# modular-ngp/phys-autodiff

Measured on NVIDIA B200. Metric: grid points/sec, fused MLP + finite-difference physics loss, higher is better.
Workload: dtype f32

## Files before the change

phys_autodiff_b200/csrc/capi.cu:

```cuda
#include "../../include/physad_b200.h"
#include "deep_grad_kernels.cuh"
#include "deep_kernels.cuh"
#include "deep_tangent_kernels.cuh"
#include "deep_tc_kernels.cuh"
#include "dense_kernels.cuh"
#include "grad_kernels.cuh"
#include "stage_kernels.cuh"
#include "tangent_grad_kernels.cuh"
#include "tangent_kernels.cuh"

#include <algorithm>
#include <cstdio>
#include <cstdlib>
#include <cstring>
#include <string>
#include <unordered_map>
#include <vector>

using namespace physad;

namespace {

thread_local std::string g_err;

int fail(int code, const std::string& msg) {
    g_err = msg;
    return code;
}

#define CU(expr)                                                                                   \
    do {                                                                                           \
        cudaError_t e_ = (expr);                                                                   \
        if (e_ != cudaSuccess)                                                                     \
            return fail(int(e_), std::string(#expr) + ": " + cudaGetErrorString(e_));              \
    } while (0)

}

struct physad_ctx {
    int device = 0;
    int sm_count = 0;
    cudaStream_t stream = nullptr;
    physad_mlp_config cfg{4, 0, 4, 1};
    bool has_weights = false;
// ... 93 lines not shown
    physad_slab r{0, g->nz};
    if (s) r = *s;
    if (r.z_begin < 0 || r.z_end > g->nz || r.z_begin > r.z_end) return fail(PHYSAD_E_INVALID, "slab outside the grid");
    *out = r;
    return 0;
}

float inv2(float h) { return float(1.0 / (2.0 * double(h))); }
double inv2d(float h) { return 1.0 / (2.0 * double(h)); }

int template_h(int H) { return H <= 32 ? 32 : (H <= 64 ? 64 : (H <= 128 ? 128 : 0)); }

template <int H>
void fill_const(const physad_ctx* c, const float tcoord[3], MlpConst<H>& k) {
    const int h_rt = c->cfg.H;
    auto W1 = [&](int h, int col) { return h < h_rt ? c->W1[size_t(h) * 4 + col] : 0.f; };
    auto B1 = [&](int h) { return h < h_rt ? c->b1[h] : 0.f; };
    auto W2 = [&](int o, int h) { return h < h_rt ? c->W2[size_t(o) * h_rt + h] : 0.f; };
    auto PT = [&](int h, int s) { volatile float p = W1(h, 3) * tcoord[s]; return float(p); };
    for (int q = 0; q < H / 2; ++q) {
        const int h0 = 2 * q, h1 = 2 * q + 1;
        k.b1p[q] = make_float2(B1(h0), B1(h1));
        k.w0s[q] = make_float2(W1(h1, 0), W1(h0, 0));
        k.w1s[q] = make_float2(W1(h1, 1), W1(h0, 1));
        k.w2s[q] = make_float2(W1(h1, 2), W1(h0, 2));
        k.ptm[q] = make_float2(PT(h0, 0), PT(h1, 0));
        k.pt0[q] = make_float2(PT(h0, 1), PT(h1, 1));
        k.ptp[q] = make_float2(PT(h0, 2), PT(h1, 2));
    }
    for (int h = 0; h < H; ++h) k.w2[h] = make_float4(W2(1, h), W2(0, h), W2(3, h), W2(2, h));
    k.b2 = make_float4(c->b2[0], c->b2[1], c->b2[2], c->b2[3]);
}

float time_coord(float t, int norm) { return norm == 1 ? t : (t + 0.5f); }

int need_4x4(const physad_ctx* c, const char* what) {
    if (!c->has_weights) return fail(PHYSAD_E_NOWEIGHTS, std::string(what) + ": no weights set");
    if (c->cfg.In != 4 || c->cfg.Out != 4)
        return fail(PHYSAD_E_UNSUPPORTED, std::string(what) + ": grid paths need In = Out = 4 (src/mlp_grid.cpp:69-80)");
    if (template_h(c->cfg.H) == 0) return fail(PHYSAD_E_UNSUPPORTED, std::string(what) + ": H > 128 not built");
    return 0;
}

float host_axis_coord(int i, int n, bool m1p1) {
    if (n <= 1) return 0.0f;
    volatile float u = float(i) / float(n - 1);
    volatile float two_u = 2.f * u;
    return m1p1 ? two_u - 1.f : float(u);
}

int ensure_coord_tables(physad_ctx* c, const physad_grid* g, cudaStream_t st) {
    const int key[5] = {g->nx, g->ny, g->nz, c->cfg.norm, 1};
    auto& t = c->tab;
    if (std::memcmp(key, t.key, sizeof(key)) == 0) return 0;
    const bool m1p1 = c->cfg.norm == 1;
    const size_t nf = size_t(g->nx) + g->ny + g->nz;
    std::vector<float> host(nf);
    for (int i = 0; i < g->nx; ++i) host[i] = host_axis_coord(i, g->nx, m1p1);
    for (int i = 0; i < g->ny; ++i) host[g->nx + i] = host_axis_coord(i, g->ny, m1p1);
    for (int i = 0; i < g->nz; ++i) host[g->nx + g->ny + i] = host_axis_coord(i, g->nz, m1p1);
    if (nf > t.cap) {
        if (t.dev) CU(cudaFree(t.dev));
        t.dev = nullptr; t.cap = 0;
        CU(cudaMalloc(&t.dev, nf * sizeof(float)));
        t.cap = nf;
    }
// ... 43 lines not shown

int build_fused_plan(physad_ctx* c, const physad_grid* g, const physad_slab& s, int TX, int TY, long long slots,
                     cudaStream_t st) {
    if (int rc = ensure_coord_tables(c, g, st)) return rc;
    auto& p = c->plan;
    p.cxs = c->tab.dev;
    p.cys = p.cxs + g->nx;
    p.czs = p.cys + g->ny;
    const int key[10] = {g->nx, g->ny, g->nz, s.z_begin, s.z_end, c->cfg.norm, TX, TY, int(slots), 1};
    if (std::memcmp(key, p.key, sizeof(key)) == 0) return 0;
    const int tiles = ((g->nx + TX - 1) / TX) * ((g->ny + TY - 1) / TY), nzl = s.z_end - s.z_begin;
    const long long want = std::min<long long>(slots, (long long)tiles * nzl);
    const std::vector<int> ranges = balanced_ranges(tiles, nzl, want, 0.9);
    const size_t bytes = ranges.size() * sizeof(int);
    if (bytes > p.cap) {
        if (p.dev) CU(cudaFree(p.dev));
        p.dev = nullptr; p.cap = 0;
        CU(cudaMalloc(&p.dev, bytes));
        p.cap = bytes;
    }
    CU(cudaMemcpyAsync(p.dev, ranges.data(), bytes, cudaMemcpyHostToDevice, st));
    CU(cudaStreamSynchronize(st));
    p.ranges = reinterpret_cast<const int*>(p.dev);
    p.blocks = int(ranges.size()) - 1;
    std::memcpy(p.key, key, sizeof(key));
    return 0;
}

template <int H, int P, int TYB, int UNROLL, int MINB, bool PACKED, bool SPLITBAR, bool DPRES>
int launch_fused_d(physad_ctx* c, const physad_grid* g, const physad_slab& s, const float tc[3], bool xchg, double* acc,
                   float* const R[4], cudaStream_t st, int blocks_per_sm_cap = 0) {
    constexpr int TX = 32, TY = TYB * P;
    auto kern = k_fused_mlp_phys_loss<H, P, TYB, UNROLL, MINB, PACKED, SPLITBAR, DPRES>;
    const size_t smem = size_t(4) * 4 * (TX + 2) * (TY + 2) * sizeof(float);
    static const long long env_blocks = getenv("PHYSAD_FUSED_BLOCKS") ? atoll(getenv("PHYSAD_FUSED_BLOCKS")) : 0;
    int& per_sm = c->blocks_per_sm[reinterpret_cast<const void*>(kern)];
    if (per_sm == 0) {
        CU(cudaFuncSetAttribute(kern, cudaFuncAttributeMaxDynamicSharedMemorySize, int(smem)));
        int q = 0;
        CU(cudaOccupancyMaxActiveBlocksPerMultiprocessor(&q, kern, 32 * TYB, smem));
        if (q < 1) return fail(PHYSAD_E_UNSUPPORTED, "fused kernel does not fit on an SM");
        per_sm = q;
    }
    const int tiles_x = (g->nx + TX - 1) / TX, tiles_y = (g->ny + TY - 1) / TY;
    const int bps = blocks_per_sm_cap > 0 ? std::min(per_sm, blocks_per_sm_cap) : per_sm;
    const long long slots = env_blocks > 0 ? env_blocks : (long long)bps * c->sm_count;
    if (int rc = build_fused_plan(c, g, s, TX, TY, slots, st)) return rc;
    const long long blocks = c->plan.blocks;
    FusedArgs a{};
    a.nx = g->nx; a.ny = g->ny; a.nz = g->nz;
    a.z_begin = s.z_begin; a.z_end = s.z_end;
    a.tiles_x = tiles_x; a.tiles_y = tiles_y;
    a.cxs = c->plan.cxs; a.cys = c->plan.cys; a.czs = c->plan.czs; a.ranges = c->plan.ranges;
    a.m1p1 = c->cfg.norm == 1; a.periodic = g->periodic != 0;
    a.inv2dt = inv2(g->dt); a.inv2hx = inv2(g->hx); a.inv2hy = inv2(g->hy); a.inv2hz = inv2(g->hz);
    a.inv2dt_d = inv2d(g->dt); a.inv2hx_d = inv2d(g->hx); a.inv2hy_d = inv2d(g->hy); a.inv2hz_d = inv2d(g->hz);
    if (int rc = ensure_partials(c, size_t(blocks))) return rc;
    a.partials = c->partials; a.ticket = c->ticket; a.acc_out = acc;
    for (int k = 0; k < 4; ++k) a.R[k] = R[k];
    if (xchg) {
        a.x.rank = c->xrank; a.x.world = c->xworld; a.x.epoch = c->xepoch + 1;
        for (int p = 0; p < XCHG_MAX_RANKS; ++p) a.x.peer[p] = c->xpeer[p];
    }
    a.status = c->d_status;
    if (c->want_host_seq) { a.host_res = c->d_res; a.host_seq = c->want_host_seq; }
    if (c->trace && blocks <= c->trace_blocks) a.trace = c->trace;
    MlpConst<H> k;
    fill_const<H>(c, tc, k);
    kern<<<unsigned(blocks), 32 * TYB, smem, st>>>(k, a);
    CU(cudaGetLastError());
    c->launches++;
    if (xchg) c->xepoch++;
    return 0;
}

template <int H, int P, int TYB, int UNROLL, int MINB, bool PACKED, bool SPLITBAR = false>
int launch_fused_t(physad_ctx* c, const physad_grid* g, const physad_slab& s, const float tc[3], bool xchg, double* acc,
                   float* const R[4], cudaStream_t st, int blocks_per_sm_cap = 0) {
    return launch_fused_d<H, P, TYB, UNROLL, MINB, PACKED, SPLITBAR, false>(c, g, s, tc, xchg, acc, R, st, blocks_per_sm_cap);
}

template <int H, bool DPRES>
int launch_fused_default(physad_ctx* c, const physad_grid* g, const physad_slab& s, const float tc[3], bool xchg,
                         double* acc, float* const R[4], cudaStream_t st) {
    const long long tile_planes = (long long)((g->nx + 31) / 32) * ((g->ny + 63) / 64) * (s.z_end - s.z_begin);
    if (tile_planes < 12LL * c->sm_count)
        return launch_fused_d<H, 4, 8, 2, 2, true, true, DPRES>(c, g, s, tc, xchg, acc, R, st, 1);
// ... 41 lines not shown
    switch (template_h(c->cfg.H)) {
        case 32: return launch_fused_h<32>(c, g, s, tc, xchg, acc, R, st);
        case 64: return launch_fused_h<64>(c, g, s, tc, xchg, acc, R, st);
        case 128: return launch_fused_h<128>(c, g, s, tc, xchg, acc, R, st);
    }
    return fail(PHYSAD_E_UNSUPPORTED, "H > 128 not built");
}

template <int H, bool FIELDS>
int launch_grid_t(physad_ctx* c, const physad_grid* g, const physad_slab& s, const float tc[3], GridInferArgs a,
                  cudaStream_t st, int dtype = PHYSAD_F32) {
    const int nzl = s.z_end - s.z_begin;
    if (nzl == 0) return 0;
    if (nzl > 65535) return fail(PHYSAD_E_UNSUPPORTED, "grid MLP kernels: more than 65535 planes per call");
    if (int rc = ensure_coord_tables(c, g, st)) return rc;
    a.cxs = c->tab.dev; a.cys = a.cxs + g->nx; a.czs = a.cys + g->ny;
    MlpConst<H> k;
    fill_const<H>(c, tc, k);
    const dim3 grid(unsigned((g->nx + 31) / 32), unsigned((g->ny + 31) / 32), unsigned(nzl));
    if (FIELDS && dtype == PHYSAD_F16) k_mlp_grid<H, FIELDS, 2, __half><<<grid, 256, 0, st>>>(k, a);
    else if (FIELDS && dtype == PHYSAD_BF16) k_mlp_grid<H, FIELDS, 2, __nv_bfloat16><<<grid, 256, 0, st>>>(k, a);
    else k_mlp_grid<H, FIELDS, 2><<<grid, 256, 0, st>>>(k, a);
    c->launches++;
    CU(cudaGetLastError());
    return 0;
}

template <bool FIELDS>
int launch_grid(physad_ctx* c, const physad_grid* g, const physad_slab& s, const float tc[3], GridInferArgs a,
                cudaStream_t st, int dtype = PHYSAD_F32) {
    a.nx = g->nx; a.ny = g->ny; a.nz = g->nz;
    a.z_begin = s.z_begin; a.z_end = s.z_end;
    a.m1p1 = c->cfg.norm == 1;
    switch (template_h(c->cfg.H)) {
        case 32: return launch_grid_t<32, FIELDS>(c, g, s, tc, a, st, dtype);
        case 64: return launch_grid_t<64, FIELDS>(c, g, s, tc, a, st, dtype);
        case 128: return launch_grid_t<128, FIELDS>(c, g, s, tc, a, st, dtype);
    }
    return fail(PHYSAD_E_UNSUPPORTED, "H > 128 not built");
}

template <bool WRITE_R, bool REDUCE, bool SCALE>
int launch_phys(physad_ctx* c, const physad_grid* g_in, PhysArgs a, cudaStream_t st, int slab_planes = -1, int dtype = PHYSAD_F32) {
    physad_grid gl = *g_in;
    if (slab_planes >= 0) gl.nz = slab_planes;
    const physad_grid* g = &gl;
    if (g->nz == 0) {
        if (REDUCE) CU(cudaMemsetAsync(a.acc_out, 0, 2 * sizeof(double), st));
        return 0;
    }
    a.nx = g->nx; a.ny = g->ny; a.nz = g->nz; a.periodic = g->periodic != 0;
    a.inv2dt = inv2(g->dt); a.inv2hx = inv2(g->hx); a.inv2hy = inv2(g->hy); a.inv2hz = inv2(g->hz);
    a.inv2dt_d = inv2d(g->dt); a.inv2hx_d = inv2d(g->hx); a.inv2hy_d = inv2d(g->hy); a.inv2hz_d = inv2d(g->hz);
    a.inv1hx_d = 1.0 / double(g->hx); a.inv1hy_d = 1.0 / double(g->hy); a.inv1hz_d = 1.0 / double(g->hz);
    a.inv1hx = float(a.inv1hx_d); a.inv1hy = float(a.inv1hy_d); a.inv1hz = float(a.inv1hz_d);
    const bool upwind = c->advection == 1;
    static const bool no_v4 = getenv("PHYSAD_NO_V4") != nullptr;
    bool v4 = !upwind && !no_v4 && g->nx % 4 == 0 && (g->nx >= 128 || dtype != PHYSAD_F32);
    const void* ptrs[12] = {a.s_m, a.s_0, a.s_p, a.u_m, a.u_0, a.u_p, a.R[0], a.R[1], a.R[2], a.R[3], a.halo_lo, a.halo_hi};
    for (int k = 0; k < 12; ++k) v4 = v4 && (uintptr_t(ptrs[k]) % ((dtype != PHYSAD_F32 && (k < 6 || k >= 10)) ? 8 : 16) == 0);
    v4 = v4 && (size_t(g->nx) * g->ny * g->nz) % 4 == 0;
    if (dtype != PHYSAD_F32 && (!v4 || SCALE || c->exact_residuals))
        return fail(PHYSAD_E_UNSUPPORTED, "16-bit fields: need nx % 4 == 0, 8-byte aligned arrays, the central scheme and fp32 residual arithmetic");
    if (v4) {
        const unsigned tx = unsigned((g->nx + 255) / 256), ty = unsigned((g->ny + V4_THREADS / 64 - 1) / (V4_THREADS / 64));
        if (ty > 65535u) return fail(PHYSAD_E_UNSUPPORTED, "phys kernels: ny > 131070");
// ... 1584 lines not shown
```

phys_autodiff_b200/csrc/fused_loss.cuh:

```cuda
#pragma once
#include <type_traits>

#include "mlp_eval.cuh"

namespace physad {

constexpr int XCHG_MAX_RANKS = 8;

struct XSlot {
    double a, b;
    unsigned long long flag;
    unsigned long long pad;
};

struct XchgArgs {
    int rank, world;
    unsigned long long epoch;
    XSlot* peer[XCHG_MAX_RANKS];
};

__device__ __forceinline__ void st_release_sys(unsigned long long* p, unsigned long long v) {
    asm volatile("st.release.sys.global.u64 [%0], %1;" ::"l"(p), "l"(v) : "memory");
}
__device__ __forceinline__ unsigned long long ld_acquire_sys(const unsigned long long* p) {
// ... 42 lines not shown
    double a, b;
    unsigned long long status;
    unsigned long long seq;
};

struct ReduceSink {
    const XchgArgs* x = nullptr;
    HostResult* host = nullptr;
    unsigned long long host_seq = 0;
    unsigned int* status = nullptr;
};

constexpr int TRACE_SLOTS = 18;
__device__ __forceinline__ unsigned long long globaltimer_ns() {
    unsigned long long t;
    asm volatile("mov.u64 %0, %%globaltimer;" : "=l"(t));
    return t;
}
__device__ __forceinline__ unsigned int smid() {
    unsigned int r;
    asm volatile("mov.u32 %0, %%smid;" : "=r"(r));
    return r;
}

struct FusedArgs {
    int nx, ny, nz;
    int z_begin, z_end;
    int tiles_x, tiles_y;
    const float* cxs;
    const float* cys;
    const float* czs;
    const int* ranges;
    int m1p1, periodic;
    float inv2dt, inv2hx, inv2hy, inv2hz;
    double inv2dt_d, inv2hx_d, inv2hy_d, inv2hz_d;
    double2* partials;
    unsigned int* ticket;
    double* acc_out;
    float* R[4];
    XchgArgs x;
    HostResult* host_res;
    unsigned long long host_seq;
    unsigned int* status;
    unsigned long long* trace;
};

__device__ __forceinline__ double warp_sum(double v) {
#pragma unroll
    for (int o = 16; o > 0; o >>= 1) v += __shfl_xor_sync(0xffffffffu, v, o);
    return v;
}

template <int NWARPS>
__device__ __forceinline__ void grid_reduce2_lin(double a, double b, double2* partials, unsigned int* ticket, double* out,
                                                 double2* s_red, unsigned int* s_flag, unsigned int block_lin,
                                                 unsigned int nblocks, const ReduceSink* sink = nullptr) {
    const int lane = threadIdx.x & 31, wid = threadIdx.x >> 5;
    a = warp_sum(a);
    b = warp_sum(b);
    if (lane == 0) s_red[wid] = make_double2(a, b);
    __syncthreads();
    if (threadIdx.x == 0) {
        double sa = 0.0, sb = 0.0;
#pragma unroll
        for (int i = 0; i < NWARPS; ++i) { sa += s_red[i].x; sb += s_red[i].y; }
        partials[block_lin] = make_double2(sa, sb);
// ... 43 lines not shown
    grid_reduce2_lin<NWARPS>(a, b, partials, ticket, out, s_red, s_flag, blockIdx.x, gridDim.x, sink);
}

static __global__ void k_xchg_only(const __grid_constant__ XchgArgs x, double* out, HostResult* host, unsigned long long host_seq,
                            unsigned int* status) {
    double a = 0.0, b = 0.0;
    const bool ok = xchg_allreduce2(x, a, b);
    if (threadIdx.x == 0) {
        out[0] = a; out[1] = b;
        if (!ok && status) *status = 1u;
        if (host) {
            host->a = a; host->b = b; host->status = ok ? 0ull : 1ull;
            __threadfence_system();
            st_release_sys(&host->seq, host_seq);
        }
    }
}

__device__ __forceinline__ unsigned smem_u32(const void* p) { return unsigned(__cvta_generic_to_shared(p)); }
__device__ __forceinline__ void mbar_init(unsigned long long* bar, unsigned count) {
    asm volatile("mbarrier.init.shared::cta.b64 [%0], %1;" ::"r"(smem_u32(bar)), "r"(count) : "memory");
}
__device__ __forceinline__ void mbar_arrive(unsigned long long* bar) {
    asm volatile("{ .reg .b64 st; mbarrier.arrive.shared::cta.b64 st, [%0]; }" ::"r"(smem_u32(bar)) : "memory");
}
__device__ __forceinline__ void mbar_wait(unsigned long long* bar, unsigned parity) {
    unsigned ok;
    do {
        asm volatile("{ .reg .pred p; mbarrier.try_wait.parity.shared::cta.b64 p, [%1], %2; selp.u32 %0, 1, 0, p; }"
                     : "=r"(ok) : "r"(smem_u32(bar)), "r"(parity) : "memory");
    } while (!ok);
}

template <int H, int P, int TYB, int UNROLL, int MINB, bool PACKED, bool SPLITBAR = false, bool DPRES = false>
__global__ void __launch_bounds__(32 * TYB, MINB)
k_fused_mlp_phys_loss(const __grid_constant__ MlpConst<H> w, const FusedArgs a) {
    constexpr int TX = 32, TY = TYB * P, NWARPS = TYB;
    static_assert((NWARPS & (NWARPS - 1)) == 0, "warps per block must be a power of two");
    constexpr int SX = TX + 2, SY = TY + 2, CH = SX * SY, PLANE = 4 * CH, NB = 4;
    constexpr int RING = 2 * TX + 2 * TY, NTASK = (RING + 31) / 32;
    extern __shared__ float smem[];
    float* buf = smem;
    __shared__ double2 s_red[NWARPS];
    __shared__ unsigned int s_flag;
    __shared__ unsigned long long s_bar[2];
    auto stamp = [&](int slot) {
        if (a.trace != nullptr && threadIdx.x == 0) {
            unsigned long long* t = a.trace + (size_t(blockIdx.x) * TRACE_SLOTS + slot) * 2;
            t[0] = globaltimer_ns();
            t[1] = (unsigned long long)clock64();
        }
    };
    stamp(0);
    if (SPLITBAR) {
        if (threadIdx.x == 0) { mbar_init(&s_bar[0], NWARPS); mbar_init(&s_bar[1], NWARPS); }
        __syncthreads();
    }

    const int tx = threadIdx.x & 31, ty = threadIdx.x >> 5;
    const bool per = a.periodic != 0;

    const int nzl = a.z_end - a.z_begin;
    const long long W = (long long)a.tiles_x * a.tiles_y * nzl;
    (void)W;
    const long long w_end = a.ranges[blockIdx.x + 1];
    long long wpos = a.ranges[blockIdx.x];
    double acc_s = 0.0, acc_u = 0.0;
    int kbuf = 0;
    int seg = 0;
    if (a.trace != nullptr && threadIdx.x == 0) {
        unsigned long long* t = a.trace + (size_t(blockIdx.x) * TRACE_SLOTS + 15) * 2;
        t[0] = smid();
        t[1] = (unsigned long long)(w_end - wpos);
    }
    stamp(1);

  while (wpos < w_end) {
    const int tile = int(wpos / nzl);
    const int zs = int(wpos - (long long)tile * nzl);
    const int nplanes = int(w_end - wpos < (long long)(nzl - zs) ? w_end - wpos : (long long)(nzl - zs));
    wpos += nplanes;
    const int zc0 = a.z_begin + zs;
    const int x0 = (tile % a.tiles_x) * TX, y0 = (tile / a.tiles_x) * TY;

    const int gx = x0 + tx;
    const float cx = __ldg(a.cxs + bc_index(gx, a.nx, per));
    float cy[P];
    bool live[P];
#pragma unroll
    for (int j = 0; j < P; ++j) {
        const int gy = y0 + ty + j * TYB;
        cy[j] = __ldg(a.cys + bc_index(gy, a.ny, per));
        live[j] = gx < a.nx && gy < a.ny;
    }
    using real = typename std::conditional<DPRES, double, float>::type;
    const real i2t = DPRES ? real(a.inv2dt_d) : real(a.inv2dt), i2x = DPRES ? real(a.inv2hx_d) : real(a.inv2hx);
    const real i2y = DPRES ? real(a.inv2hy_d) : real(a.inv2hy), i2z = DPRES ? real(a.inv2hz_d) : real(a.inv2hz);
    real dT[P][4];
#pragma unroll
    for (int j = 0; j < P; ++j)
#pragma unroll
        for (int c = 0; c < 4; ++c) dT[j][c] = real(0);

    if (seg < 4) stamp(2 + 3 * seg);
    float cz_next = __ldg(a.czs + bc_index(zc0 - 1, a.nz, per));
    for (int k = 0; k <= nplanes + 1; ++k, ++kbuf) {
        const int zk = zc0 - 1 + k;
        const float cz = cz_next;
        cz_next = __ldg(a.czs + bc_index(zk + 1, a.nz, per));
        if (k == 1 && seg < 4) stamp(3 + 3 * seg);
        float* pl = buf + (kbuf & (NB - 1)) * PLANE;
        const bool halo_plane = (k == 0) || (k == nplanes + 1);
        real dTn[P][4];
        if (halo_plane) {
            float y[P][1][4];
            mlp_eval<H, 1, P, UNROLL, PACKED>(w, cx, cy, cz, y);
#pragma unroll
            for (int j = 0; j < P; ++j) {
                const int o = (1 + ty + j * TYB) * SX + 1 + tx;
#pragma unroll
                for (int c = 0; c < 4; ++c) { pl[c * CH + o] = y[j][0][c]; dTn[j][c] = real(0); }
            }
        } else {
            float y[P][3][4];
            mlp_eval<H, 3, P, UNROLL, PACKED>(w, cx, cy, cz, y);
#pragma unroll
            for (int j = 0; j < P; ++j) {
                const int o = (1 + ty + j * TYB) * SX + 1 + tx;
#pragma unroll
                for (int c = 0; c < 4; ++c) {
                    pl[c * CH + o] = y[j][1][c];
                    dTn[j][c] = central_diff(y[j][2][c], y[j][0][c], i2t);
                }
            }
            {
                static_assert(NTASK <= NWARPS, "one ring task per warp and plane");
                const int i = (ty - kbuf) & (NWARPS - 1);
                if (i < NTASK) {
                    const int r = i * 32 + tx;
                    int xx, yy;
                    if (r < TX) { xx = 1 + r; yy = 0; }
                    else if (r < 2 * TX) { xx = 1 + r - TX; yy = SY - 1; }
                    else if (r < 2 * TX + TY) { xx = 0; yy = 1 + r - 2 * TX; }
                    else { xx = SX - 1; yy = 1 + r - 2 * TX - TY; }
                    if (r >= RING) { xx = 0; yy = 0; }
                    const float rcx = __ldg(a.cxs + bc_index(x0 - 1 + xx, a.nx, per));
                    const float rc[1] = {__ldg(a.cys + bc_index(y0 - 1 + yy, a.ny, per))};
                    float yr[1][1][4];
                    mlp_eval<H, 1, 1, UNROLL, PACKED>(w, rcx, rc, cz, yr);
                    if (r < RING) {
#pragma unroll
                        for (int c = 0; c < 4; ++c) pl[c * CH + yy * SX + xx] = yr[0][0][c];
                    }
                }
            }
        }
        if (SPLITBAR) {
            __syncwarp();
            if (tx == 0) mbar_arrive(&s_bar[kbuf & 1]);
            if (kbuf >= 1) mbar_wait(&s_bar[(kbuf - 1) & 1], unsigned((kbuf - 1) >> 1) & 1u);
        } else {
            __syncthreads();
        }
        if (k >= 2) {
            const float* pc = buf + ((kbuf - 1) & (NB - 1)) * PLANE;
            const float* pm = buf + ((kbuf - 2) & (NB - 1)) * PLANE;
            const float* pp = pl;
            const int zl = zk - 1 - a.z_begin;
#pragma unroll
            for (int j = 0; j < P; ++j) {
// ... 41 lines not shown
```

phys_autodiff_b200/csrc/mlp_eval.cuh:

```cuda
#pragma once
#include <cuda_runtime.h>

namespace physad {

template <int H>
struct MlpConst {
    static_assert(H % 2 == 0, "hidden units are processed in pairs");
    float2 b1p[H / 2];
    float2 w0s[H / 2];
    float2 w1s[H / 2];
    float2 w2s[H / 2];
    float2 ptm[H / 2];
    float2 pt0[H / 2];
    float2 ptp[H / 2];
    float4 w2[H];
    float4 b2;
};

__device__ __forceinline__ float relu_ref(float s) {
    return fmaxf(s, 0.f);
}

__device__ __forceinline__ float axis_coord(int i, int n, bool m1p1) {
    if (n <= 1) return 0.f;
// ... 10 lines not shown
}

typedef unsigned long long f32x2;

__device__ __forceinline__ f32x2 pack2(float lo, float hi) {
    f32x2 r;
    asm("mov.b64 %0, {%1, %2};" : "=l"(r) : "f"(lo), "f"(hi));
    return r;
}
__device__ __forceinline__ void unpack2(f32x2 v, float& lo, float& hi) {
    asm("mov.b64 {%0, %1}, %2;" : "=f"(lo), "=f"(hi) : "l"(v));
}
__device__ __forceinline__ f32x2 mul2_rn(f32x2 a, f32x2 b) {
    f32x2 r;
    asm("mul.rn.f32x2 %0, %1, %2;" : "=l"(r) : "l"(a), "l"(b));
    return r;
}
__device__ __forceinline__ f32x2 add2_rn_swapped(f32x2 acc, f32x2 p) {
    float lo, hi;
    unpack2(p, lo, hi);
    f32x2 r;
    asm("add.rn.f32x2 %0, %1, %2;" : "=l"(r) : "l"(acc), "l"(pack2(hi, lo)));
    return r;
}

__device__ __forceinline__ f32x2 add2_rn(f32x2 a, f32x2 b) {
    f32x2 r;
    asm("add.rn.f32x2 %0, %1, %2;" : "=l"(r) : "l"(a), "l"(b));
    return r;
}
__device__ __forceinline__ f32x2 pack2(float2 v) { return pack2(v.x, v.y); }
__device__ __forceinline__ f32x2 bcast2(float v) { return pack2(v, v); }

template <int H, int NS, int P, int UNROLL, bool PACKED>
__device__ __forceinline__ void mlp_eval(const MlpConst<H>& w, float cx, const float (&cy)[P], float cz,
                                         float (&y)[P][NS][4]) {
    const float4 b2 = w.b2;
    f32x2 q01[P][NS], q23[P][NS];
#pragma unroll
    for (int j = 0; j < P; ++j)
#pragma unroll
        for (int s = 0; s < NS; ++s) {
            if (PACKED) {
                q01[j][s] = pack2(b2.x, b2.y);
                q23[j][s] = pack2(b2.z, b2.w);
            } else {
                y[j][s][0] = b2.x; y[j][s][1] = b2.y; y[j][s][2] = b2.z; y[j][s][3] = b2.w;
            }
        }
#pragma unroll UNROLL
    for (int q = 0; q < H / 2; ++q) {
        const float2 b1p = w.b1p[q], w0s = w.w0s[q], w1s = w.w1s[q], w2s = w.w2s[q];
        const float2 tm = w.ptm[q], t0 = w.pt0[q], tp = w.ptp[q];
        const float4 ca = w.w2[2 * q], cb = w.w2[2 * q + 1];
        if (PACKED) {
            const f32x2 sx = add2_rn_swapped(pack2(b1p), mul2_rn(pack2(w0s), bcast2(cx)));
            const f32x2 mz = mul2_rn(pack2(w2s), bcast2(cz));
            const f32x2 ca10 = pack2(ca.x, ca.y), ca32 = pack2(ca.z, ca.w);
            const f32x2 cb10 = pack2(cb.x, cb.y), cb32 = pack2(cb.z, cb.w);
#pragma unroll
            for (int j = 0; j < P; ++j) {
                const f32x2 sxy = add2_rn_swapped(sx, mul2_rn(pack2(w1s), bcast2(cy[j])));
                const f32x2 sxyz = add2_rn_swapped(sxy, mz);
#pragma unroll
                for (int s = 0; s < NS; ++s) {
                    const float2 pt = (NS == 1) ? t0 : (s == 0 ? tm : (s == 1 ? t0 : tp));
                    float v0, v1;
                    unpack2(add2_rn(sxyz, pack2(pt)), v0, v1);
                    const f32x2 a0 = bcast2(relu_ref(v0)), a1 = bcast2(relu_ref(v1));
                    q01[j][s] = add2_rn_swapped(q01[j][s], mul2_rn(a0, ca10));
                    q23[j][s] = add2_rn_swapped(q23[j][s], mul2_rn(a0, ca32));
                    q01[j][s] = add2_rn_swapped(q01[j][s], mul2_rn(a1, cb10));
                    q23[j][s] = add2_rn_swapped(q23[j][s], mul2_rn(a1, cb32));
                }
            }
        } else {
#pragma unroll
            for (int e = 0; e < 2; ++e) {
                const float b1 = e ? b1p.y : b1p.x, w0 = e ? w0s.x : w0s.y, w1 = e ? w1s.x : w1s.y, w2 = e ? w2s.x : w2s.y;
                const float4 c = e ? cb : ca;
                const float sx = __fadd_rn(b1, __fmul_rn(w0, cx));
                const float mz = __fmul_rn(w2, cz);
#pragma unroll
                for (int j = 0; j < P; ++j) {
                    const float sxyz = __fadd_rn(__fadd_rn(sx, __fmul_rn(w1, cy[j])), mz);
#pragma unroll
                    for (int s = 0; s < NS; ++s) {
                        const float2 pt2 = (NS == 1) ? t0 : (s == 0 ? tm : (s == 1 ? t0 : tp));
                        const float act = relu_ref(__fadd_rn(sxyz, e ? pt2.y : pt2.x));
                        y[j][s][0] = __fadd_rn(y[j][s][0], __fmul_rn(c.y, act));
                        y[j][s][1] = __fadd_rn(y[j][s][1], __fmul_rn(c.x, act));
                        y[j][s][2] = __fadd_rn(y[j][s][2], __fmul_rn(c.w, act));
                        y[j][s][3] = __fadd_rn(y[j][s][3], __fmul_rn(c.z, act));
                    }
                }
            }
        }
    }
    if (PACKED) {
#pragma unroll
        for (int j = 0; j < P; ++j)
#pragma unroll
            for (int s = 0; s < NS; ++s) {
                unpack2(q01[j][s], y[j][s][0], y[j][s][1]);
                unpack2(q23[j][s], y[j][s][2], y[j][s][3]);
            }
    }
}

__device__ __forceinline__ float central_diff(float plus, float minus, float inv2h) {
    return __fmul_rn(__fsub_rn(plus, minus), inv2h);
}
__device__ __forceinline__ double central_diff(float plus, float minus, double inv2h) {
    return __dmul_rn(__dsub_rn(double(plus), double(minus)), inv2h);
}

__device__ __forceinline__ void point_residual(const float (&f)[4], const float (&gx)[4], const float (&gy)[4],
                                               const float (&gz)[4], const float (&dT)[4], float (&R)[4]) {
    const float div = __fadd_rn(__fadd_rn(gx[1], gy[2]), gz[3]);
#pragma unroll
    for (int c = 0; c < 4; ++c) {
        const float adv = __fmaf_rn(f[3], gz[c], __fmaf_rn(f[2], gy[c], __fmul_rn(f[1], gx[c])));
        R[c] = __fadd_rn(dT[c], adv);
    }
    R[0] = __fmaf_rn(f[0], div, R[0]);
}

__device__ __forceinline__ void point_residual(const float (&f)[4], const double (&gx)[4], const double (&gy)[4],
                                               const double (&gz)[4], const double (&dT)[4], float (&R)[4]) {
    const double ux = double(f[1]), uy = double(f[2]), uz = double(f[3]);
    const double div = __dadd_rn(__dadd_rn(gx[1], gy[2]), gz[3]);
#pragma unroll
    for (int c = 0; c < 4; ++c) {
        const double adv = __dadd_rn(__dadd_rn(__dmul_rn(ux, gx[c]), __dmul_rn(uy, gy[c])), __dmul_rn(uz, gz[c]));
        const double r = __dadd_rn(dT[c], adv);
        R[c] = float(c == 0 ? __dadd_rn(r, __dmul_rn(double(f[0]), div)) : r);
    }
}

template <typename T>
__device__ __forceinline__ void point_residual_upwind(const float (&f)[4], const float (&xm)[4], const float (&xp)[4],
                                                      const float (&ym)[4], const float (&yp)[4], const float (&zm)[4],
// ... 16 lines not shown
```

phys_autodiff_b200/csrc/stage_kernels.cuh:

```cuda
#pragma once
#include <cuda_bf16.h>
#include <cuda_fp16.h>

#include "fused_loss.cuh"

namespace physad {

__device__ __forceinline__ float4 ldg4(const float* p) { return __ldg(reinterpret_cast<const float4*>(p)); }
__device__ __forceinline__ float4 ldg4(const __half* p) {
    const uint2 v = __ldg(reinterpret_cast<const uint2*>(p));
    const float2 a = __half22float2(*reinterpret_cast<const __half2*>(&v.x)), b = __half22float2(*reinterpret_cast<const __half2*>(&v.y));
    return make_float4(a.x, a.y, b.x, b.y);
}
__device__ __forceinline__ float4 ldg4(const __nv_bfloat16* p) {
    const uint2 v = __ldg(reinterpret_cast<const uint2*>(p));
    const float2 a = __bfloat1622float2(*reinterpret_cast<const __nv_bfloat162*>(&v.x));
    const float2 b = __bfloat1622float2(*reinterpret_cast<const __nv_bfloat162*>(&v.y));
    return make_float4(a.x, a.y, b.x, b.y);
}
__device__ __forceinline__ float ldg1(const float* p) { return __ldg(p); }
__device__ __forceinline__ float ldg1(const __half* p) { return __half2float(__ldg(p)); }
__device__ __forceinline__ float ldg1(const __nv_bfloat16* p) { return __bfloat162float(__ldg(p)); }
__device__ __forceinline__ void st1(float* p, float v) { *p = v; }
__device__ __forceinline__ void st1(__half* p, float v) { *p = __float2half_rn(v); }
__device__ __forceinline__ void st1(__nv_bfloat16* p, float v) { *p = __float2bfloat16_rn(v); }


struct GridInferArgs {
    int nx, ny, nz;
    int z_begin, z_end;
    int m1p1;
    const float* cxs; const float* cys; const float* czs;
    float4* out_aos;
    float* sigma[3];
    float* u[3];
    size_t cstride;
};

template <int H, bool FIELDS, int UNROLL, typename E = float>
__global__ void __launch_bounds__(256) k_mlp_grid(const __grid_constant__ MlpConst<H> w, const GridInferArgs a) {
    constexpr int P = 4;
    const int x = blockIdx.x * 32 + (threadIdx.x & 31);
    const int y0 = blockIdx.y * 32 + (threadIdx.x >> 5);
    const int z = a.z_begin + blockIdx.z;
    const size_t n = a.cstride ? a.cstride : size_t(a.z_end - a.z_begin) * a.ny * a.nx;
    const float cx = __ldg(a.cxs + min(x, a.nx - 1));
    const float cz = __ldg(a.czs + z);
    float cy[P];
#pragma unroll
    for (int j = 0; j < P; ++j) cy[j] = __ldg(a.cys + min(y0 + 8 * j, a.ny - 1));
    if (FIELDS) {
        float o[P][3][4];
        mlp_eval<H, 3, P, UNROLL, true>(w, cx, cy, cz, o);
#pragma unroll
        for (int j = 0; j < P; ++j) {
            const int y = y0 + 8 * j;
            if (x < a.nx && y < a.ny) {
                const size_t i = (size_t(blockIdx.z) * a.ny + y) * a.nx + x;
#pragma unroll
                for (int s = 0; s < 3; ++s) {
                    E* ps = reinterpret_cast<E*>(a.sigma[s]);
                    E* pu = reinterpret_cast<E*>(a.u[s]);
                    st1(ps + i, o[j][s][0]);
                    st1(pu + i, o[j][s][1]);
                    st1(pu + n + i, o[j][s][2]);
                    st1(pu + 2 * n + i, o[j][s][3]);
                }
            }
        }
    } else {
        float o[P][1][4];
        mlp_eval<H, 1, P, UNROLL, true>(w, cx, cy, cz, o);
#pragma unroll
        for (int j = 0; j < P; ++j) {
            const int y = y0 + 8 * j;
            if (x < a.nx && y < a.ny)
                a.out_aos[(size_t(blockIdx.z) * a.ny + y) * a.nx + x] = make_float4(o[j][0][0], o[j][0][1], o[j][0][2], o[j][0][3]);
        }
    }
}

__global__ void __launch_bounds__(256) k_mlp_forward_4x4(const float4* __restrict__ x, const float* __restrict__ W1,
                                                         const float* __restrict__ b1, const float* __restrict__ W2,
                                                         const float* __restrict__ b2, float4* __restrict__ y, size_t B,
                                                         int H) {
    extern __shared__ float4 sw[];
    float4* s_a = sw;
    float4* s_b = sw + H;
    float* s_c = reinterpret_cast<float*>(sw + 2 * H);
    for (int h = threadIdx.x; h < H; h += blockDim.x) {
        s_a[h] = make_float4(b1[h], W1[h * 4 + 0], W1[h * 4 + 1], W1[h * 4 + 2]);
        s_b[h] = make_float4(W1[h * 4 + 3], W2[h], W2[H + h], W2[2 * H + h]);
        s_c[h] = W2[3 * H + h];
    }
    __syncthreads();
    const size_t i = size_t(blockIdx.x) * blockDim.x + threadIdx.x;
    if (i >= B) return;
    const float4 p = x[i];
    float o0 = b2[0], o1 = b2[1], o2 = b2[2], o3 = b2[3];
#pragma unroll 4
    for (int h = 0; h < H; ++h) {
        const float4 a = s_a[h], c = s_b[h];
        const float d = s_c[h];
        float s = __fadd_rn(a.x, __fmul_rn(a.y, p.x));
        s = __fadd_rn(s, __fmul_rn(a.z, p.y));
// ... 247 lines not shown
```

Baseline: 15.76 billion.

## Precompute per-tile first-layer partial sums in shared memory for packed fused MLP

In the packed path, the first-layer pre-activation terms are now precomputed into shared-memory tables. The x term is built per column and for the halo edges, the y term per warp row, and the z term per plane. The MLP inner loop then only adds table entries, where before it recomputed the w0*x + w1*y + w2*z products for every hidden unit and point. Ring halo tasks are restructured to reuse the same tables, and with two points per lane when the ring is large. This adds shared memory per block and extra barriers, which may cut occupancy and adds shared-memory load traffic in the hot loop.

```diff
diff --git a/phys_autodiff_b200/csrc/capi.cu b/phys_autodiff_b200/csrc/capi.cu
--- a/phys_autodiff_b200/csrc/capi.cu
+++ b/phys_autodiff_b200/csrc/capi.cu
@@ -278,7 +278,7 @@
                    float* const R[4], cudaStream_t st, int blocks_per_sm_cap = 0) {
     constexpr int TX = 32, TY = TYB * P;
     auto kern = k_fused_mlp_phys_loss<H, P, TYB, UNROLL, MINB, PACKED, SPLITBAR, DPRES>;
-    const size_t smem = size_t(4) * 4 * (TX + 2) * (TY + 2) * sizeof(float);
+    const size_t smem = fused_smem_bytes<H, P, TYB, PACKED>();
     static const long long env_blocks = getenv("PHYSAD_FUSED_BLOCKS") ? atoll(getenv("PHYSAD_FUSED_BLOCKS")) : 0;
     int& per_sm = c->blocks_per_sm[reinterpret_cast<const void*>(kern)];
     if (per_sm == 0) {
diff --git a/phys_autodiff_b200/csrc/fused_loss.cuh b/phys_autodiff_b200/csrc/fused_loss.cuh
--- a/phys_autodiff_b200/csrc/fused_loss.cuh
+++ b/phys_autodiff_b200/csrc/fused_loss.cuh
@@ -207,15 +207,67 @@
     } while (!ok);
 }
 
+template <int H, int P, int TYB, bool PACKED>
+constexpr size_t fused_smem_bytes() {
+    return sizeof(float) * (size_t(4) * 4 * (32 + 2) * (TYB * P + 2) + (PACKED ? size_t(H) * (32 + 2 + TYB * P + TYB + 4) : 0));
+}
+
+template <int H, int NP, int TY, int UNROLL>
+__device__ __forceinline__ void ring_task(const MlpConst<H>& w, const FusedArgs& a, int task, int y0, bool per,
+                                          const float4* sxt, const float4* sxe, const float4* mz, float* pl) {
+    constexpr int TX = 32, SX = TX + 2, SY = TY + 2, CH = SX * SY;
+    const int tx = threadIdx.x & 31;
+    const float4* sp[NP];
+    int ss[NP], o[NP];
+    float cy[NP];
+    bool keep[NP];
+#pragma unroll
+    for (int j = 0; j < NP; ++j) {
+        int xx, yy;
+        if (task == 0) {
+            xx = 1 + tx; yy = j ? SY - 1 : 0;
+            keep[j] = true;
+            sp[j] = sxt + tx; ss[j] = TX;
+        } else {
+            const int c = (task - 1) * 32 * NP + j * 32 + tx;
+            keep[j] = c < 2 * TY;
+            if (c < TY) { xx = 0; yy = 1 + c; }
+            else if (c < 2 * TY) { xx = SX - 1; yy = 1 + c - TY; }
+            else { xx = 0; yy = 0; }
+            sp[j] = sxe + (xx == 0 ? 0 : H / 4); ss[j] = 1;
+        }
+        cy[j] = __ldg(a.cys + bc_index(y0 - 1 + yy, a.ny, per));
+        o[j] = yy * SX + xx;
+    }
+    auto pre = [&](int q2, int e, int j) {
+        const float4 s = sp[j][q2 * ss[j]];
+        return add2_rn_swapped(e ? pack2(s.z, s.w) : pack2(s.x, s.y), mul2_rn(pack2(w.w1s[2 * q2 + e]), bcast2(cy[j])));
+    };
+    float y[NP][1][4];
+    mlp_eval_pre<H, 1, NP, UNROLL>(w, pre, mz, y);
+#pragma unroll
+    for (int j = 0; j < NP; ++j)
+        if (keep[j]) {
+#pragma unroll
+            for (int c = 0; c < 4; ++c) pl[c * CH + o[j]] = y[j][0][c];
+        }
+}
+
 template <int H, int P, int TYB, int UNROLL, int MINB, bool PACKED, bool SPLITBAR = false, bool DPRES = false>
 __global__ void __launch_bounds__(32 * TYB, MINB)
 k_fused_mlp_phys_loss(const __grid_constant__ MlpConst<H> w, const FusedArgs a) {
     constexpr int TX = 32, TY = TYB * P, NWARPS = TYB;
     static_assert((NWARPS & (NWARPS - 1)) == 0, "warps per block must be a power of two");
     constexpr int SX = TX + 2, SY = TY + 2, CH = SX * SY, PLANE = 4 * CH, NB = 4;
-    constexpr int RING = 2 * TX + 2 * TY, NTASK = (RING + 31) / 32;
-    extern __shared__ float smem[];
+    constexpr int RING = 2 * TX + 2 * TY, SP = 2 * TY >= 64 ? 2 : 1;
+    constexpr int NTASK = PACKED ? 1 + (2 * TY + 32 * SP - 1) / (32 * SP) : (RING + 31) / 32;
+    constexpr int Q4 = H / 4;
+    extern __shared__ __align__(16) float smem[];
     float* buf = smem;
+    float4* sxt = reinterpret_cast<float4*>(smem + NB * PLANE);
+    float4* sxe = sxt + Q4 * TX;
+    float4* wtab = sxe + 2 * Q4;
+    float2* sw1 = reinterpret_cast<float2*>(wtab + NWARPS * (P + 1) * Q4);
     __shared__ double2 s_red[NWARPS];
     __shared__ unsigned int s_flag;
     __shared__ unsigned long long s_bar[2];
@@ -227,8 +279,14 @@
         }
     };
     stamp(0);
-    if (SPLITBAR) {
-        if (threadIdx.x == 0) { mbar_init(&s_bar[0], NWARPS); mbar_init(&s_bar[1], NWARPS); }
+    if (PACKED) {
+        for (int i = threadIdx.x; i < 2 * H; i += 32 * NWARPS) {
+            const int q = i % (H / 2), r = i / (H / 2);
+            sw1[i] = r == 0 ? w.b1p[q] : r == 1 ? w.w0s[q] : r == 2 ? w.w1s[q] : w.w2s[q];
+        }
+    }
+    if (SPLITBAR || PACKED) {
+        if (SPLITBAR && threadIdx.x == 0) { mbar_init(&s_bar[0], NWARPS); mbar_init(&s_bar[1], NWARPS); }
         __syncthreads();
     }
 
@@ -278,6 +336,31 @@
         for (int c = 0; c < 4; ++c) dT[j][c] = real(0);
 
     if (seg < 4) stamp(2 + 3 * seg);
+    float4* const w1yw = wtab + ty * (P + 1) * Q4;
+    float4* const mzw = w1yw + P * Q4;
+    if (PACKED) {
+        if (SPLITBAR) __syncthreads();
+        for (int q = ty; q < H / 2; q += NWARPS) {
+            float lo, hi;
+            unpack2(add2_rn_swapped(pack2(sw1[q]), mul2_rn(pack2(sw1[H / 2 + q]), bcast2(cx))), lo, hi);
+            reinterpret_cast<float2*>(sxt)[((q >> 1) * TX + tx) * 2 + (q & 1)] = make_float2(lo, hi);
+        }
+        for (int i = threadIdx.x; i < H; i += 32 * NWARPS) {
+            const int e = i / (H / 2), q = i % (H / 2);
+            const float ex = __ldg(a.cxs + bc_index(e ? x0 + TX : x0 - 1, a.nx, per));
+            float lo, hi;
+            unpack2(add2_rn_swapped(pack2(sw1[q]), mul2_rn(pack2(sw1[H / 2 + q]), bcast2(ex))), lo, hi);
+            reinterpret_cast<float2*>(sxe)[e * H / 2 + q] = make_float2(lo, hi);
+        }
+#pragma unroll
+        for (int j = 0; j < P; ++j)
+            for (int q = tx; q < H / 2; q += 32) {
+                float lo, hi;
+                unpack2(mul2_rn(pack2(sw1[H + q]), bcast2(cy[j])), lo, hi);
+                reinterpret_cast<float2*>(w1yw)[j * H / 2 + q] = make_float2(hi, lo);
+            }
+        __syncthreads();
+    }
     float cz_next = __ldg(a.czs + bc_index(zc0 - 1, a.nz, per));
     for (int k = 0; k <= nplanes + 1; ++k, ++kbuf) {
         const int zk = zc0 - 1 + k;
@@ -286,10 +369,23 @@
         if (k == 1 && seg < 4) stamp(3 + 3 * seg);
         float* pl = buf + (kbuf & (NB - 1)) * PLANE;
         const bool halo_plane = (k == 0) || (k == nplanes + 1);
+        if (PACKED) {
+            for (int q = tx; q < H / 2; q += 32) {
+                float lo, hi;
+                unpack2(mul2_rn(pack2(sw1[3 * H / 2 + q]), bcast2(cz)), lo, hi);
+                reinterpret_cast<float2*>(mzw)[q] = make_float2(hi, lo);
+            }
+            __syncwarp();
+        }
+        auto pre_tile = [&](int q2, int e, int j) {
+            const float4 s = sxt[q2 * TX + tx], v = w1yw[j * Q4 + q2];
+            return e ? add2_rn(pack2(s.z, s.w), pack2(v.z, v.w)) : add2_rn(pack2(s.x, s.y), pack2(v.x, v.y));
+        };
         real dTn[P][4];
         if (halo_plane) {
             float y[P][1][4];
-            mlp_eval<H, 1, P, UNROLL, PACKED>(w, cx, cy, cz, y);
+            if constexpr (PACKED) mlp_eval_pre<H, 1, P, UNROLL>(w, pre_tile, mzw, y);
+            else mlp_eval<H, 1, P, UNROLL, PACKED>(w, cx, cy, cz, y);
 #pragma unroll
             for (int j = 0; j < P; ++j) {
                 const int o = (1 + ty + j * TYB) * SX + 1 + tx;
@@ -298,7 +394,8 @@
             }
         } else {
             float y[P][3][4];
-            mlp_eval<H, 3, P, UNROLL, PACKED>(w, cx, cy, cz, y);
+            if constexpr (PACKED) mlp_eval_pre<H, 3, P, UNROLL>(w, pre_tile, mzw, y);
+            else mlp_eval<H, 3, P, UNROLL, PACKED>(w, cx, cy, cz, y);
 #pragma unroll
             for (int j = 0; j < P; ++j) {
                 const int o = (1 + ty + j * TYB) * SX + 1 + tx;
@@ -308,9 +405,14 @@
                     dTn[j][c] = central_diff(y[j][2][c], y[j][0][c], i2t);
                 }
             }
-            {
-                static_assert(NTASK <= NWARPS, "one ring task per warp and plane");
-                const int i = (ty - kbuf) & (NWARPS - 1);
+            static_assert(NTASK <= NWARPS, "one ring task per warp and plane");
+            const int i = (ty - kbuf) & (NWARPS - 1);
+            if constexpr (PACKED && SP == 2) {
+                if (i < NTASK) ring_task<H, 2, TY, UNROLL>(w, a, i, y0, per, sxt, sxe, mzw, pl);
+            } else if constexpr (PACKED) {
+                if (i == 0) ring_task<H, 2, TY, UNROLL>(w, a, i, y0, per, sxt, sxe, mzw, pl);
+                else if (i < NTASK) ring_task<H, 1, TY, UNROLL>(w, a, i, y0, per, sxt, sxe, mzw, pl);
+            } else {
                 if (i < NTASK) {
                     const int r = i * 32 + tx;
                     int xx, yy;
diff --git a/phys_autodiff_b200/csrc/mlp_eval.cuh b/phys_autodiff_b200/csrc/mlp_eval.cuh
--- a/phys_autodiff_b200/csrc/mlp_eval.cuh
+++ b/phys_autodiff_b200/csrc/mlp_eval.cuh
@@ -142,6 +142,56 @@
     }
 }
 
+template <int H, int NS, int P, int UNROLL, class Pre>
+__device__ __forceinline__ void mlp_eval_pre(const MlpConst<H>& w, const Pre& pre, const float4* mz4, float (&y)[P][NS][4]) {
+    static_assert(H % 4 == 0 && UNROLL % 2 == 0, "the tables are read two hidden-unit pairs at a time");
+    constexpr int U2 = UNROLL / 2;
+    const float4 b2 = w.b2;
+    f32x2 q01[P][NS], q23[P][NS];
+#pragma unroll
+    for (int j = 0; j < P; ++j)
+#pragma unroll
+        for (int s = 0; s < NS; ++s) {
+            q01[j][s] = pack2(b2.x, b2.y);
+            q23[j][s] = pack2(b2.z, b2.w);
+        }
+#pragma unroll U2
+    for (int q2 = 0; q2 < H / 4; ++q2) {
+        const float4 m = mz4[q2];
+#pragma unroll
+        for (int e = 0; e < 2; ++e) {
+            const int q = 2 * q2 + e;
+            const float2 tm = w.ptm[q], t0 = w.pt0[q], tp = w.ptp[q];
+            const float4 ca = w.w2[2 * q], cb = w.w2[2 * q + 1];
+            const f32x2 mz = e ? pack2(m.z, m.w) : pack2(m.x, m.y);
+            const f32x2 ca10 = pack2(ca.x, ca.y), ca32 = pack2(ca.z, ca.w);
+            const f32x2 cb10 = pack2(cb.x, cb.y), cb32 = pack2(cb.z, cb.w);
+#pragma unroll
+            for (int j = 0; j < P; ++j) {
+                const f32x2 sxyz = add2_rn(pre(q2, e, j), mz);
+#pragma unroll
+                for (int s = 0; s < NS; ++s) {
+                    const float2 pt = (NS == 1) ? t0 : (s == 0 ? tm : (s == 1 ? t0 : tp));
+                    float v0, v1;
+                    unpack2(add2_rn(sxyz, pack2(pt)), v0, v1);
+                    const f32x2 a0 = bcast2(relu_ref(v0)), a1 = bcast2(relu_ref(v1));
+                    q01[j][s] = add2_rn_swapped(q01[j][s], mul2_rn(a0, ca10));
+                    q23[j][s] = add2_rn_swapped(q23[j][s], mul2_rn(a0, ca32));
+                    q01[j][s] = add2_rn_swapped(q01[j][s], mul2_rn(a1, cb10));
+                    q23[j][s] = add2_rn_swapped(q23[j][s], mul2_rn(a1, cb32));
+                }
+            }
+        }
+    }
+#pragma unroll
+    for (int j = 0; j < P; ++j)
+#pragma unroll
+        for (int s = 0; s < NS; ++s) {
+            unpack2(q01[j][s], y[j][s][0], y[j][s][1]);
+            unpack2(q23[j][s], y[j][s][2], y[j][s][3]);
+        }
+}
+
 __device__ __forceinline__ float central_diff(float plus, float minus, float inv2h) {
     return __fmul_rn(__fsub_rn(plus, minus), inv2h);
 }
```

Result: faster. 16.10 billion, median of 6 (+2.2%).

## Skip layer-2 accumulation for hidden units dead across the warp via ballot

Applied to the files above, without the earlier changes.

Adds a warp-wide vote on hidden-unit pre-activations so that when a hidden unit's ReLU is non-positive for every point in the warp, its second-layer multiply-adds are skipped. The vote runs only on pairs flagged dead on the previous tile, with a full reset every few tiles, and only when the host confirms W2 is finite and b2 has no negative zeros, to keep results bitwise exact. This targets redundant FMA work in sparse-activation regimes. The cost is extra reduce_or syncs, a split code path and the loss of unrolling (UNROLL forced to 1) in the fused kernel.

```diff
diff --git a/phys_autodiff_b200/csrc/capi.cu b/phys_autodiff_b200/csrc/capi.cu
--- a/phys_autodiff_b200/csrc/capi.cu
+++ b/phys_autodiff_b200/csrc/capi.cu
@@ -10,6 +10,7 @@
 #include "tangent_kernels.cuh"
 
 #include <algorithm>
+#include <cmath>
 #include <cstdio>
 #include <cstdlib>
 #include <cstring>
@@ -169,6 +170,14 @@
     k.b2 = make_float4(c->b2[0], c->b2[1], c->b2[2], c->b2[3]);
 }
 
+bool layer2_skip_exact(const physad_ctx* c) {
+    for (int o = 0; o < 4; ++o)
+        if (c->b2[o] == 0.f && std::signbit(c->b2[o])) return false;
+    for (size_t i = 0; i < size_t(4) * c->cfg.H; ++i)
+        if (!std::isfinite(c->W2[i])) return false;
+    return true;
+}
+
 float time_coord(float t, int norm) { return norm == 1 ? t : (t + 0.5f); }
 
 int need_4x4(const physad_ctx* c, const char* what) {
@@ -299,6 +308,7 @@
     a.tiles_x = tiles_x; a.tiles_y = tiles_y;
     a.cxs = c->plan.cxs; a.cys = c->plan.cys; a.czs = c->plan.czs; a.ranges = c->plan.ranges;
     a.m1p1 = c->cfg.norm == 1; a.periodic = g->periodic != 0;
+    a.skip_ok = layer2_skip_exact(c);
     a.inv2dt = inv2(g->dt); a.inv2hx = inv2(g->hx); a.inv2hy = inv2(g->hy); a.inv2hz = inv2(g->hz);
     a.inv2dt_d = inv2d(g->dt); a.inv2hx_d = inv2d(g->hx); a.inv2hy_d = inv2d(g->hy); a.inv2hz_d = inv2d(g->hz);
     if (int rc = ensure_partials(c, size_t(blocks))) return rc;
@@ -406,6 +416,7 @@
     a.nx = g->nx; a.ny = g->ny; a.nz = g->nz;
     a.z_begin = s.z_begin; a.z_end = s.z_end;
     a.m1p1 = c->cfg.norm == 1;
+    a.skip_ok = layer2_skip_exact(c);
     switch (template_h(c->cfg.H)) {
         case 32: return launch_grid_t<32, FIELDS>(c, g, s, tc, a, st, dtype);
         case 64: return launch_grid_t<64, FIELDS>(c, g, s, tc, a, st, dtype);
diff --git a/phys_autodiff_b200/csrc/fused_loss.cuh b/phys_autodiff_b200/csrc/fused_loss.cuh
--- a/phys_autodiff_b200/csrc/fused_loss.cuh
+++ b/phys_autodiff_b200/csrc/fused_loss.cuh
@@ -98,6 +98,7 @@
     const float* czs;
     const int* ranges;
     int m1p1, periodic;
+    int skip_ok;
     float inv2dt, inv2hx, inv2hy, inv2hz;
     double inv2dt_d, inv2hx_d, inv2hy_d, inv2hz_d;
     double2* partials;
@@ -214,6 +215,9 @@
     static_assert((NWARPS & (NWARPS - 1)) == 0, "warps per block must be a power of two");
     constexpr int SX = TX + 2, SY = TY + 2, CH = SX * SY, PLANE = 4 * CH, NB = 4;
     constexpr int RING = 2 * TX + 2 * TY, NTASK = (RING + 31) / 32;
+    constexpr bool VOTE = PACKED && !DPRES;
+    constexpr int REVOTE = 8;
+    unsigned long long vote_pairs = ~0ull;
     extern __shared__ float smem[];
     float* buf = smem;
     __shared__ double2 s_red[NWARPS];
@@ -298,7 +302,8 @@
             }
         } else {
             float y[P][3][4];
-            mlp_eval<H, 3, P, UNROLL, PACKED>(w, cx, cy, cz, y);
+            if (k == 1 || (k & (REVOTE - 1)) == 0) vote_pairs = ~0ull;
+            mlp_eval<H, 3, P, VOTE ? 1 : UNROLL, PACKED, VOTE>(w, cx, cy, cz, y, a.skip_ok != 0, &vote_pairs);
 #pragma unroll
             for (int j = 0; j < P; ++j) {
                 const int o = (1 + ty + j * TYB) * SX + 1 + tx;
diff --git a/phys_autodiff_b200/csrc/mlp_eval.cuh b/phys_autodiff_b200/csrc/mlp_eval.cuh
--- a/phys_autodiff_b200/csrc/mlp_eval.cuh
+++ b/phys_autodiff_b200/csrc/mlp_eval.cuh
@@ -66,9 +66,27 @@
 __device__ __forceinline__ f32x2 pack2(float2 v) { return pack2(v.x, v.y); }
 __device__ __forceinline__ f32x2 bcast2(float v) { return pack2(v, v); }
 
-template <int H, int NS, int P, int UNROLL, bool PACKED>
+__device__ __forceinline__ float max3(float a, float b, float c) {
+    float r;
+    asm("max.f32 %0, %1, %2, %3;" : "=f"(r) : "f"(a), "f"(b), "f"(c));
+    return r;
+}
+
+template <int N>
+__device__ __forceinline__ float max_of(const float (&v)[N]) {
+    float m = v[0];
+#pragma unroll
+    for (int i = 1; i < N; i += 2) m = (i + 1 < N) ? max3(m, v[i], v[i + 1 < N ? i + 1 : i]) : fmaxf(m, v[i]);
+    return m;
+}
+
+template <int H, int NS, int P, int UNROLL, bool PACKED, bool VOTE = false>
 __device__ __forceinline__ void mlp_eval(const MlpConst<H>& w, float cx, const float (&cy)[P], float cz,
-                                         float (&y)[P][NS][4]) {
+                                         float (&y)[P][NS][4], bool skip_ok = false,
+                                         unsigned long long* vote_pairs = nullptr) {
+    static_assert(H / 2 <= 64, "one vote bit per hidden pair");
+    const unsigned long long want = vote_pairs != nullptr ? *vote_pairs : ~0ull;
+    unsigned long long dead = 0ull;
     const float4 b2 = w.b2;
     f32x2 q01[P][NS], q23[P][NS];
 #pragma unroll
@@ -82,6 +100,7 @@
                 y[j][s][0] = b2.x; y[j][s][1] = b2.y; y[j][s][2] = b2.z; y[j][s][3] = b2.w;
             }
         }
+    static_assert(PACKED || !VOTE, "only the packed path votes");
 #pragma unroll UNROLL
     for (int q = 0; q < H / 2; ++q) {
         const float2 b1p = w.b1p[q], w0s = w.w0s[q], w1s = w.w1s[q], w2s = w.w2s[q];
@@ -92,20 +111,57 @@
             const f32x2 mz = mul2_rn(pack2(w2s), bcast2(cz));
             const f32x2 ca10 = pack2(ca.x, ca.y), ca32 = pack2(ca.z, ca.w);
             const f32x2 cb10 = pack2(cb.x, cb.y), cb32 = pack2(cb.z, cb.w);
-#pragma unroll
-            for (int j = 0; j < P; ++j) {
-                const f32x2 sxy = add2_rn_swapped(sx, mul2_rn(pack2(w1s), bcast2(cy[j])));
-                const f32x2 sxyz = add2_rn_swapped(sxy, mz);
-#pragma unroll
-                for (int s = 0; s < NS; ++s) {
-                    const float2 pt = (NS == 1) ? t0 : (s == 0 ? tm : (s == 1 ? t0 : tp));
-                    float v0, v1;
-                    unpack2(add2_rn(sxyz, pack2(pt)), v0, v1);
-                    const f32x2 a0 = bcast2(relu_ref(v0)), a1 = bcast2(relu_ref(v1));
-                    q01[j][s] = add2_rn_swapped(q01[j][s], mul2_rn(a0, ca10));
-                    q23[j][s] = add2_rn_swapped(q23[j][s], mul2_rn(a0, ca32));
-                    q01[j][s] = add2_rn_swapped(q01[j][s], mul2_rn(a1, cb10));
-                    q23[j][s] = add2_rn_swapped(q23[j][s], mul2_rn(a1, cb32));
+            if (!VOTE || !skip_ok || !((want >> q) & 1ull)) {
+#pragma unroll
+                for (int j = 0; j < P; ++j) {
+                    const f32x2 sxy = add2_rn_swapped(sx, mul2_rn(pack2(w1s), bcast2(cy[j])));
+                    const f32x2 sxyz = add2_rn_swapped(sxy, mz);
+#pragma unroll
+                    for (int s = 0; s < NS; ++s) {
+                        const float2 pt = (NS == 1) ? t0 : (s == 0 ? tm : (s == 1 ? t0 : tp));
+                        float v0, v1;
+                        unpack2(add2_rn(sxyz, pack2(pt)), v0, v1);
+                        const f32x2 a0 = bcast2(relu_ref(v0)), a1 = bcast2(relu_ref(v1));
+                        q01[j][s] = add2_rn_swapped(q01[j][s], mul2_rn(a0, ca10));
+                        q23[j][s] = add2_rn_swapped(q23[j][s], mul2_rn(a0, ca32));
+                        q01[j][s] = add2_rn_swapped(q01[j][s], mul2_rn(a1, cb10));
+                        q23[j][s] = add2_rn_swapped(q23[j][s], mul2_rn(a1, cb32));
+                    }
+                }
+            } else {
+                float v0[P * NS], v1[P * NS];
+#pragma unroll
+                for (int j = 0; j < P; ++j) {
+                    const f32x2 sxy = add2_rn_swapped(sx, mul2_rn(pack2(w1s), bcast2(cy[j])));
+                    const f32x2 sxyz = add2_rn_swapped(sxy, mz);
+#pragma unroll
+                    for (int s = 0; s < NS; ++s) {
+                        const float2 pt = (NS == 1) ? t0 : (s == 0 ? tm : (s == 1 ? t0 : tp));
+                        unpack2(add2_rn(sxyz, pack2(pt)), v0[j * NS + s], v1[j * NS + s]);
+                    }
+                }
+                const unsigned live =
+                    __reduce_or_sync(0xffffffffu, (max_of(v0) > 0.f ? 1u : 0u) | (max_of(v1) > 0.f ? 2u : 0u));
+                if (live != 3u) dead |= 1ull << q;
+                if (live & 1u) {
+#pragma unroll
+                    for (int j = 0; j < P; ++j)
+#pragma unroll
+                        for (int s = 0; s < NS; ++s) {
+                            const f32x2 a0 = bcast2(relu_ref(v0[j * NS + s]));
+                            q01[j][s] = add2_rn_swapped(q01[j][s], mul2_rn(a0, ca10));
+                            q23[j][s] = add2_rn_swapped(q23[j][s], mul2_rn(a0, ca32));
+                        }
+                }
+                if (live & 2u) {
+#pragma unroll
+                    for (int j = 0; j < P; ++j)
+#pragma unroll
+                        for (int s = 0; s < NS; ++s) {
+                            const f32x2 a1 = bcast2(relu_ref(v1[j * NS + s]));
+                            q01[j][s] = add2_rn_swapped(q01[j][s], mul2_rn(a1, cb10));
+                            q23[j][s] = add2_rn_swapped(q23[j][s], mul2_rn(a1, cb32));
+                        }
                 }
             }
         } else {
@@ -131,6 +187,7 @@
             }
         }
     }
+    if (vote_pairs != nullptr) *vote_pairs = dead;
     if (PACKED) {
 #pragma unroll
         for (int j = 0; j < P; ++j)
diff --git a/phys_autodiff_b200/csrc/stage_kernels.cuh b/phys_autodiff_b200/csrc/stage_kernels.cuh
--- a/phys_autodiff_b200/csrc/stage_kernels.cuh
+++ b/phys_autodiff_b200/csrc/stage_kernels.cuh
@@ -30,6 +30,7 @@
     int nx, ny, nz;
     int z_begin, z_end;
     int m1p1;
+    int skip_ok;
     const float* cxs; const float* cys; const float* czs;
     float4* out_aos;
     float* sigma[3];
@@ -51,7 +52,7 @@
     for (int j = 0; j < P; ++j) cy[j] = __ldg(a.cys + min(y0 + 8 * j, a.ny - 1));
     if (FIELDS) {
         float o[P][3][4];
-        mlp_eval<H, 3, P, UNROLL, true>(w, cx, cy, cz, o);
+        mlp_eval<H, 3, P, UNROLL, true, true>(w, cx, cy, cz, o, a.skip_ok != 0);
 #pragma unroll
         for (int j = 0; j < P; ++j) {
             const int y = y0 + 8 * j;
@@ -70,7 +71,7 @@
         }
     } else {
         float o[P][1][4];
-        mlp_eval<H, 1, P, UNROLL, true>(w, cx, cy, cz, o);
+        mlp_eval<H, 1, P, UNROLL, true, true>(w, cx, cy, cz, o, a.skip_ok != 0);
 #pragma unroll
         for (int j = 0; j < P; ++j) {
             const int y = y0 + 8 * j;
```

New measurement: 15.74 billion before, 17.42 billion after (median of 6 runs). 1.11x the previous value.
